# CoderWZW/ARLib

Hardware: AMD Instinct MI355X
Metric: BPR-train interactions/sec (LightGCN d=64 L=3 + BPR + Adam, B=2048) (higher is better)
Workload: dtype f32

## Files before the change

### arlib_amd/csrc/arl_kernels.hip

```cpp
#include <hip/hip_runtime.h>
#include <stdint.h>
#include <math.h>
#include <stdio.h>
#include "arlib_amd.h"
#include <type_traits>

#define ARL_LAUNCH_CHECK()                                  \
    do {                                                    \
        hipError_t e__ = hipGetLastError();                 \
        if (e__ != hipSuccess) return (int)e__;             \
    } while (0)

namespace {

constexpr int kWave = 64;
constexpr int kBlock = 256;
constexpr int kWavesPerBlock = kBlock / kWave;

__device__ __forceinline__ float wave_sum(float v) {
#pragma unroll
    for (int off = 32; off > 0; off >>= 1) v += __shfl_xor(v, off);
    return v;
}

// ... 324 lines not shown
        const int r = rows[t];
        const int begin = A.rowptr[r], end = A.rowptr[r + 1];
        const int per = (end - begin + sp - 1) / sp;
        const int b = begin + k * per, e = min(end, b + per);
        float4 a = make_float4(0.f, 0.f, 0.f, 0.f);
        if (b < e) a = spmm_gather<LPR, 4>(A.col, A.val, b, e, X, d, lane);
        a = group_reduce<LPR>(a);
        if (lane < LPR && q * 4 < d) *reinterpret_cast<float4 *>(partial + (size_t)piece * d + q * 4) = a;
    }
}

template <int LPR>
__global__ __launch_bounds__(kBlock) void subset_pieces_finish_kernel(const float *__restrict__ partial, int n, SubsetPlan S, int d, const int32_t *__restrict__ rows,
                                                                       LayerPtrs L, float alpha, float *__restrict__ out_c, const float *__restrict__ row_weight) {
    constexpr int G = kWave / LPR;
    const int lane = threadIdx.x & (kWave - 1);
    const int g = lane / LPR, q = lane % LPR;
    const int t = blockIdx.x * kWavesPerBlock + (threadIdx.x >> 6);
    if (t >= n) return;
    const bool qact = q * 4 < d;
    const int r = rows[t];
    float4 a = make_float4(0.f, 0.f, 0.f, 0.f);
    if (g == 0 && qact)
        for (int k = 0; k < L.n; ++k) a = add4(a, *reinterpret_cast<const float4 *>(L.p[k] + (size_t)r * d + q * 4));
    const int p1 = S.offs[t + 1];
    if (qact)
        for (int p = S.offs[t] + g; p < p1; p += 8 * G) {
            float4 v[8];
#pragma unroll
            for (int u = 0; u < 8; ++u)
                if (p + u * G < p1) v[u] = *reinterpret_cast<const float4 *>(partial + (size_t)(p + u * G) * d + q * 4);
#pragma unroll
            for (int u = 0; u < 8; ++u)
                if (p + u * G < p1) a = add4(a, v[u]);
        }
    a = group_reduce<LPR>(a);
    if (lane >= LPR || !qact) return;
    const float w = row_weight ? alpha * row_weight[t] : alpha;
    *reinterpret_cast<float4 *>(out_c + (size_t)t * d + q * 4) = make_float4(w * a.x, w * a.y, w * a.z, w * a.w);
}

static bool subset_plan(void *workspace, long long n, long long nsplit, long long d, SubsetPlan *S) {
    const long long words = n * nsplit * d, tail = n + 3;
    const long long cap = (words - tail) / (d + 1);
    if (cap < n || cap > 0x7fffffffll || n > (long long)kSubsetPrepThreads * kSubsetPrepRows) return false;
    int32_t *w = (int32_t *)workspace;
    S->cap = (int)cap;
    S->piece_row = w + cap * d;
    S->meta = S->piece_row + cap;
    S->offs = S->meta + 2;
    return true;
}

__global__ __launch_bounds__(kBlock) void tables_sum_kernel(LayerPtrs L, long long n4, float alpha, float4 *__restrict__ out) {
    for (long long t = (long long)blockIdx.x * kBlock + threadIdx.x; t < n4; t += (long long)gridDim.x * kBlock) {
        float4 a = reinterpret_cast<const float4 *>(L.p[0])[t];
        for (int k = 1; k < L.n; ++k) a = add4(a, reinterpret_cast<const float4 *>(L.p[k])[t]);
        out[t] = make_float4(alpha * a.x, alpha * a.y, alpha * a.z, alpha * a.w);
    }
}

__global__ __launch_bounds__(kBlock) void mark_rows_kernel(uint8_t *__restrict__ flags, const int32_t *__restrict__ idx, int n, int value) {
    const int t = blockIdx.x * kBlock + threadIdx.x;
    if (t < n) flags[idx[t]] = (uint8_t)value;
}
__global__ __launch_bounds__(kBlock) void mark_bits_kernel(uint32_t *__restrict__ bits, const int32_t *__restrict__ idx, int n, int set) {
    const int t = blockIdx.x * kBlock + threadIdx.x;
    if (t >= n) return;
    const int i = idx[t];
    if (set) atomicOr(bits + (i >> 5), 1u << (i & 31));
    else atomicAnd(bits + (i >> 5), ~(1u << (i & 31)));
}
__global__ __launch_bounds__(kBlock) void zero_rows_kernel(float *__restrict__ dst, const int32_t *__restrict__ idx, int n, int d) {
    const int lane = threadIdx.x & 63;
    const int t = blockIdx.x * kWavesPerBlock + (threadIdx.x >> 6);
    if (t >= n) return;
    float *o = dst + (size_t)idx[t] * d;
    for (int k = lane; k < d; k += kWave) o[k] = 0.f;
}

constexpr int kOrderedWindow = 16384;

template <class RowOf, class OnHit>
__device__ __forceinline__ bool ordered_scan(int c0, int c1, int t, long long row, int lane, RowOf rowof, OnHit on_hit) {
    for (int base = c0; base < c1; base += 256) {
        long long v[4];
#pragma unroll
        for (int i = 0; i < 4; ++i) {
            const int j = base + 64 * i + lane;
            v[i] = j < c1 ? (long long)rowof(j) : -1ll;
        }
#pragma unroll
        for (int i = 0; i < 4; ++i) {
            unsigned long long m = __ballot(v[i] == row);
            const int b0 = base + 64 * i;
            if (b0 < t) {
                const int lim = t - b0;
                if (lim >= 64 ? m != 0ull : (m & ((1ull << lim) - 1ull)) != 0ull) return false;
            }
            while (m) {
                const int tt = b0 + __ffsll((long long)m) - 1;
                m &= m - 1ull;
                on_hit(tt);
            }
        }
    }
    return true;
}

template <class OnHit>
__device__ __forceinline__ bool ordered_scan_lds(const int32_t *srows, int c0, int c1, int t, int row, int lane, OnHit on_hit) {
    const int n = c1 - c0, tl = t - c0;
    for (int base = 0; base < n; base += 512) {
        int v[8];
#pragma unroll
        for (int i = 0; i < 8; ++i) {
            const int j = base + 64 * i + lane;
            v[i] = j < n ? srows[j] : -1;
        }
#pragma unroll
        for (int i = 0; i < 8; ++i) {
            unsigned long long m = __ballot(v[i] == row);
            const int b0 = base + 64 * i;
            if (b0 < tl) {
                const int lim = tl - b0;
                if (lim >= 64 ? m != 0ull : (m & ((1ull << lim) - 1ull)) != 0ull) return false;
            }
            while (m) {
                const int tt = c0 + b0 + __ffsll((long long)m) - 1;
                m &= m - 1ull;
                on_hit(tt);
            }
        }
    }
    return true;
}
template <class OnGroup>
__device__ __forceinline__ bool ordered_scan_lds_groups(const int32_t *srows, int c0, int c1, int t, int row, int lane, OnGroup on_group) {
    const int n = c1 - c0, tl = t - c0;
    for (int base = 0; base < n; base += 512) {
        int v[8];
#pragma unroll
        for (int i = 0; i < 8; ++i) {
            const int j = base + 64 * i + lane;
            v[i] = j < n ? srows[j] : -1;
        }
#pragma unroll
        for (int i = 0; i < 8; ++i) {
            const unsigned long long m = __ballot(v[i] == row);
            const int b0 = base + 64 * i;
            if (b0 < tl) {
                const int lim = tl - b0;
                if (lim >= 64 ? m != 0ull : (m & ((1ull << lim) - 1ull)) != 0ull) return false;
            }
            if (m) on_group(m, c0 + b0);
        }
    }
    return true;
}
template <class RowOf>
__device__ __forceinline__ void stage_rows(int32_t *srows, int c0, int c1, RowOf rowof) {
    for (int j = threadIdx.x; j < c1 - c0; j += kBlock) srows[j] = (int32_t)rowof(c0 + j);
    __syncthreads();
}

__global__ __launch_bounds__(kBlock) void rows_mark_dups_kernel(uint32_t *__restrict__ bits, uint32_t *__restrict__ dup, const int32_t *__restrict__ idx, int n,
                                                                 const float *__restrict__ row_scale) {
    const int t = blockIdx.x * kBlock + threadIdx.x;
    if (t >= n) return;
    if (row_scale && row_scale[t] == 0.f) return;
    const int row = idx[t];
    const uint32_t m = 1u << (row & 31);
    if (atomicOr(bits + (row >> 5), m) & m) atomicOr(dup + (row >> 5), m);
}

template <bool MARK>
__global__ __launch_bounds__(kBlock) void rows_add_ordered_kernel(float *__restrict__ dst, uint8_t *__restrict__ flags, uint32_t *__restrict__ bits,
                                                                   const int32_t *__restrict__ idx, int c0, int c1, int d,
                                                                   const float *__restrict__ src, float scale, const float *__restrict__ row_scale,
                                                                   const uint32_t *__restrict__ dup) {
    extern __shared__ int32_t srows[];
    const int lane = threadIdx.x & 63;
    const int t = c0 + blockIdx.x * kWavesPerBlock + (threadIdx.x >> 6);
    const bool valid = t < c1 && !(row_scale && row_scale[t] == 0.f);
    const int row = valid ? idx[t] : 0;
    float *o = dst + (size_t)row * d;
    const bool fast = valid && dup && !((dup[row >> 5] >> (row & 31)) & 1u);
    if (fast) {
        const float sc = row_scale ? scale * row_scale[t] : scale;
        const float *s = src + (size_t)t * d;
        for (int k = lane; k < d; k += kWave) {
#pragma clang fp contract(off)
            const float c = sc * s[k];
            o[k] = o[k] + c;
        }
        if (MARK && lane == 0) flags[row] = 1;
    }
    if (!__syncthreads_or(valid && !fast)) return;
    stage_rows(srows, c0, c1, [&](int j) { return (row_scale && row_scale[j] == 0.f) ? -1 : idx[j]; });
    if (!valid || fast) return;
    for (int k0 = 0; k0 < d; k0 += 256) {
        float acc[4];
#pragma unroll
        for (int i = 0; i < 4; ++i) { const int k = k0 + 64 * i + lane; acc[i] = k < d ? o[k] : 0.f; }
        const bool owner = ordered_scan_lds_groups(srows, c0, c1, t, row, lane, [&](unsigned long long m, int g0) {
#pragma clang fp contract(off)
            while (m) {
                int tt[4]; float x[4][4], sc[4];
#pragma unroll
                for (int q = 0; q < 4; ++q) {
                    tt[q] = -1;
                    if (m) { tt[q] = g0 + __ffsll((long long)m) - 1; m &= m - 1ull; }
                }
#pragma unroll
                for (int q = 0; q < 4; ++q) {
                    if (tt[q] < 0) continue;
                    const float *s = src + (size_t)tt[q] * d;
                    sc[q] = row_scale ? scale * row_scale[tt[q]] : scale;
#pragma unroll
                    for (int i = 0; i < 4; ++i) { const int k = k0 + 64 * i + lane; x[q][i] = k < d ? s[k] : 0.f; }
                }
#pragma unroll
                for (int q = 0; q < 4; ++q) {
                    if (tt[q] < 0) continue;
#pragma unroll
                    for (int i = 0; i < 4; ++i) { const float c = sc[q] * x[q][i]; acc[i] = acc[i] + c; }
                }
            }
        });
        if (!owner) return;
#pragma unroll
        for (int i = 0; i < 4; ++i) { const int k = k0 + 64 * i + lane; if (k < d) o[k] = acc[i]; }
    }
    if (MARK && lane == 0) {
        flags[row] = 1;
        atomicOr(bits + (row >> 5), 1u << (row & 31));
    }
}
__global__ __launch_bounds__(kBlock) void batch_rows_clear_kernel(float *__restrict__ G, uint8_t *__restrict__ flags, uint32_t *__restrict__ bits,
                                                                   const int32_t *__restrict__ idx, int n, int d, uint32_t *__restrict__ dup) {
    const int lane = threadIdx.x & 63;
    const int t = blockIdx.x * kWavesPerBlock + (threadIdx.x >> 6);
    if (t >= n) return;
    const int row = idx[t];
    float *o = G + (size_t)row * d;
    for (int k = lane; k < d; k += kWave) o[k] = 0.f;
    if (lane == 0) {
        flags[row] = 0;
        atomicAnd(bits + (row >> 5), ~(1u << (row & 31)));
        if (dup) atomicAnd(dup + (row >> 5), ~(1u << (row & 31)));
    }
}

template <int MODE>
int launch_spmm(const arl_csr *A, const float *X, int64_t d, const Epi &ep, hipStream_t st, const uint32_t *xflags = nullptr) {
    if (!A || !X || (A->n_rows > 0 && !A->rowptr) || (A->nnz > 0 && (!A->col || !A->val))) return ARL_E_NULL;
    if (d <= 0 || d > 256 || (d & 3)) return ARL_E_DIM;
    if (A->n_rows < 0 || A->n_rows > 0x7fffffffll || A->nnz > 0x7fffffffll || A->n_chunks > 0x7fffffffll) return ARL_E_RANGE;
    if (A->n_chunks > 0 && (!A->chunk_row || !A->chunk_begin || !A->chunk_end || !A->partial || A->chunk <= 0)) return ARL_E_NULL;
    if (A->n_long > 0 && (!A->long_row || !A->long_first || !A->long_count)) return ARL_E_NULL;
    if ((A->n_chunks > 0) != (A->n_long > 0)) return ARL_E_ARG;
    if (A->n_rows == 0 && A->n_chunks == 0) return ARL_OK;
    CsrDev D;
    D.n_rows = (int)A->n_rows; D.rowptr = A->rowptr; D.col = A->col; D.val = A->val;
    D.chunk = A->chunk; D.n_chunks = (int)A->n_chunks; D.chunk_row = A->chunk_row; D.chunk_begin = A->chunk_begin;
    D.chunk_end = A->chunk_end; D.n_long = (int)A->n_long; D.long_row = A->long_row; D.long_first = A->long_first;
    D.long_count = A->long_count; D.partial = A->partial;
    D.row_tasks = xflags ? reinterpret_cast<const int4 *>(A->row_tasks) : nullptr;
    const long long tasks = (long long)D.n_rows + D.n_chunks;
    const unsigned grid = (unsigned)((tasks + kWavesPerBlock - 1) / kWavesPerBlock);
    const unsigned grid_long = (unsigned)((D.n_long + kWavesPerBlock - 1) / kWavesPerBlock);
    const int di = (int)d;
#define ARL_SPMM_CASE(LPRV)                                                                              \
    do {                                                                                                 \
        if (xflags) hipLaunchKernelGGL((spmm_rows_masked_gpr_kernel<LPRV, MODE>), dim3((unsigned)((tasks + kWavesPerBlock * (kWave / LPRV) - 1) / (kWavesPerBlock * (kWave / LPRV)))), dim3(kBlock), 0, st, D, X, di, ep, xflags); \
        else hipLaunchKernelGGL((spmm_rows_kernel<LPRV, MODE>), dim3(grid), dim3(kBlock), 0, st, D, X, di, ep); \
        ARL_LAUNCH_CHECK();                                                                              \
        if (D.n_long > 0) {                                                                              \
            hipLaunchKernelGGL((spmm_long_rows_kernel<LPRV, MODE>), dim3(grid_long), dim3(kBlock), 0, st, D, di, ep); \
            ARL_LAUNCH_CHECK();                                                                          \
        }                                                                                                \
    } while (0)
    if (d <= 16) ARL_SPMM_CASE(4);
    else if (d <= 32) ARL_SPMM_CASE(8);
    else if (d <= 64) ARL_SPMM_CASE(16);
    else if (d <= 128) ARL_SPMM_CASE(32);
    else ARL_SPMM_CASE(64);
#undef ARL_SPMM_CASE
    return ARL_OK;
}

typedef float f32x32v __attribute__((ext_vector_type(32)));

struct BlockedDev {
    int n_waves;
    const int32_t *wave_ptr;
    const int32_t *wave_rows;
    const int32_t *rec_col;
    const float *rec_val;
    float *partial;
    const uint32_t *xbits;
};

template <int MODE, int CPL, int LD>
__device__ __forceinline__ void spmm_epilogue1(const Epi &ep, int row, int lane, const float *a) {
    const size_t o = (size_t)row * LD + lane * CPL;
    const bool zr = ep.Z && (!ep.zflags || ep.zflags[row]);
#pragma unroll
    for (int c = 0; c < CPL; ++c) {
        if (MODE == EPI_AXPBY) {
            float y = (ep.rscale ? ep.alpha * ep.rscale[row] : ep.alpha) * a[c];
            if (zr) y = fmaf(ep.beta, ep.Z[o + c], y);
            __builtin_nontemporal_store(y, ep.Y + o + c);
        } else if (MODE == EPI_LAYERSUM) {
            const float sv = ep.S_in[o + c];
            if (ep.Y) ep.Y[o + c] = a[c];
            ep.S[o + c] = sv + a[c];
        } else {
            float g = ep.alpha * a[c];
            if (zr) g = fmaf(ep.beta, ep.Z[o + c], g);
            float p = ep.P[o + c], m = ep.M[o + c], v = ep.V[o + c];
            m = m + (g - m) * ep.w1;
            v = v * ep.b2 + ep.w2 * g * g;
            const float denom = sqrtf(v) / ep.bc2_sqrt + ep.eps;
            p = p - ep.step_size * (m / denom);
            ep.P[o + c] = p; ep.M[o + c] = m; ep.V[o + c] = v;
        }
    }
}

constexpr int kMaskedUnr = 8;

template <int RPW, int MODE, int UNR, int CPL, int LD = 64 * CPL, bool MASKED = false>
__global__ __launch_bounds__(kBlock) void spmm_blocked64_kernel(BlockedDev P, const float *__restrict__ X, Epi ep) {
    static_assert(RPW == 16 || RPW == 32, "accumulators are 32-register vectors");
    static_assert(CPL == 1 || CPL == 2, "d = 64 (one column per lane) or d = 128 (two adjacent columns per lane)");
    const int lane = threadIdx.x & 63;
    const int w = blockIdx.x * (blockDim.x >> 6) + (threadIdx.x >> 6);
    if (w >= P.n_waves) return;
    f32x32v acc[CPL];
#pragma unroll
    for (int c = 0; c < CPL; ++c)
#pragma unroll
        for (int r = 0; r < 32; ++r) acc[c][r] = 0.f;
    const int begin = P.wave_ptr[w], end = P.wave_ptr[w + 1];
    const float *xl = X + lane * CPL;
    if (MASKED) {
        int c0 = 0, c1 = 0; unsigned w0 = 0;
        if (begin < end) c0 = __builtin_nontemporal_load(P.rec_col + begin + lane);
        if (begin + 64 < end) c1 = __builtin_nontemporal_load(P.rec_col + begin + 64 + lane);
        if (begin < end) w0 = P.xbits[((unsigned)c0 & 0xffffffu) >> 5];
        for (int base = begin; base < end; base += 64) {
            const int c_cur = c0; const unsigned w_cur = w0;
            c0 = c1;
            if (base + 128 < end) c1 = __builtin_nontemporal_load(P.rec_col + base + 128 + lane);
            if (base + 64 < end) w0 = P.xbits[((unsigned)c0 & 0xffffffu) >> 5];
            unsigned long long hits = __ballot((w_cur >> (c_cur & 31)) & 1u);
            while (hits) {
                float x[kMaskedUnr][CPL], vs[kMaskedUnr]; int cs[kMaskedUnr], js[kMaskedUnr];
#pragma unroll
                for (int t = 0; t < kMaskedUnr; ++t) {
                    js[t] = hits ? __builtin_ctzll(hits) : -1;
                    hits &= hits - 1ull;
                    if (js[t] < 0) continue;
                    cs[t] = __builtin_amdgcn_readlane(c_cur, js[t]);
                    vs[t] = P.rec_val[base + js[t]];
                    const float *src = xl + (size_t)(cs[t] & 0xffffff) * LD;
                    if (CPL == 2) { const float2 v2 = *reinterpret_cast<const float2 *>(src); x[t][0] = v2.x; x[t][CPL - 1] = v2.y; }
                    else x[t][0] = src[0];
                }
#pragma unroll
                for (int t = 0; t < kMaskedUnr; ++t) {
                    if (js[t] < 0) continue;
                    const int slot = ((unsigned)cs[t] >> 24) & 31;
#pragma unroll
                    for (int c = 0; c < CPL; ++c) acc[c][slot] = fmaf(vs[t], x[t][c], acc[c][slot]);
                }
            }
        }
    } else {
    int rc = 0; float rv = 0.f;
    if (begin < end) { rc = __builtin_nontemporal_load(P.rec_col + begin + lane); rv = __builtin_nontemporal_load(P.rec_val + begin + lane); }
    for (int base = begin; base < end; base += 64) {
        const int c_cur = rc; const float v_cur = rv;
        if (base + 64 < end) { rc = __builtin_nontemporal_load(P.rec_col + base + 64 + lane); rv = __builtin_nontemporal_load(P.rec_val + base + 64 + lane); }
#pragma unroll
        for (int j = 0; j < 64; j += UNR) {
            float x[UNR][CPL]; int cs[UNR];
#pragma unroll
            for (int t = 0; t < UNR; ++t) {
                cs[t] = __builtin_amdgcn_readlane(c_cur, j + t);
                const float *src = xl + (size_t)(cs[t] & 0xffffff) * LD;
                if (CPL == 2) { const float2 v2 = *reinterpret_cast<const float2 *>(src); x[t][0] = v2.x; x[t][CPL - 1] = v2.y; }
                else x[t][0] = src[0];
            }
#pragma unroll
            for (int t = 0; t < UNR; ++t) {
                const int slot = ((unsigned)cs[t] >> 24) & 31;
                const float v = __uint_as_float((unsigned)__builtin_amdgcn_readlane((int)__float_as_uint(v_cur), j + t));
#pragma unroll
                for (int c = 0; c < CPL; ++c) acc[c][slot] = fmaf(v, x[t][c], acc[c][slot]);
            }
        }
    }
    }
#pragma unroll
    for (int r = 0; r < RPW; ++r) {
        const int row = P.wave_rows[w * RPW + r];
        float a[CPL];
#pragma unroll
        for (int c = 0; c < CPL; ++c) a[c] = acc[c][r];
        if (row >= 0) spmm_epilogue1<MODE, CPL, LD>(ep, row, lane, a);
        else if (row < -1) {
            float *dst = P.partial + ((size_t)(-row - 2) * 64 + lane) * CPL;
#pragma unroll
            for (int c = 0; c < CPL; ++c) dst[c] = a[c];
        }
    }
}

template <int RPW, int MODE, int UNR, int CPL, int LD>
static int launch_blocked64(dim3 grid, dim3 block, hipStream_t st, const BlockedDev &D, const float *X, const Epi &ep) {
    if (D.xbits) {
        if constexpr (MODE == EPI_AXPBY) hipLaunchKernelGGL((spmm_blocked64_kernel<RPW, MODE, UNR, CPL, LD, true>), grid, block, 0, st, D, X, ep);
        else return ARL_E_ARG;
    } else hipLaunchKernelGGL((spmm_blocked64_kernel<RPW, MODE, UNR, CPL, LD, false>), grid, block, 0, st, D, X, ep);
    ARL_LAUNCH_CHECK();
    return ARL_OK;
}

template <int MODE>
int launch_spmm_blocked(const arl_blocked *P, const float *X, int64_t d, const Epi &ep, hipStream_t st, const uint32_t *xbits = nullptr) {
    if (!P || !X) return ARL_E_NULL;
    if (d != 64 && d != 128) return ARL_E_DIM;
    if (P->n_waves < 0 || P->n_waves > 0x7fffffffll / 64) return ARL_E_RANGE;
    if (P->rows_per_wave != 16 && P->rows_per_wave != 32) return ARL_E_ARG;
    if (P->n_waves == 0) return ARL_OK;
    if (!P->wave_ptr || !P->wave_rows || !P->rec_col || !P->rec_val) return ARL_E_NULL;
    if (P->n_split < 0 || P->n_split > 0x7fffffffll) return ARL_E_RANGE;
    if (P->n_split > 0 && (!P->split_row || !P->split_first || !P->split_count || !P->partial)) return ARL_E_NULL;
    BlockedDev D = {(int)P->n_waves, P->wave_ptr, P->wave_rows, P->rec_col, P->rec_val, P->partial, xbits};
    const int64_t wpg = P->waves_per_group ? P->waves_per_group : kWavesPerBlock;
    if (wpg != 1 && wpg != 2 && wpg != 4) return ARL_E_ARG;
    const dim3 grid((unsigned)((P->n_waves + wpg - 1) / wpg)), block((unsigned)(wpg * kWave));
    if (P->loads_in_flight != 16 && P->loads_in_flight != 32) return ARL_E_ARG;
    int rc;
    if (d == 128) {
        for (int half = 0; half < 2; ++half) {
            Epi e2 = ep;
            e2.ld = 128;
            const int off = 64 * half;
            if (e2.Z) e2.Z += off;
            if (e2.Y) e2.Y += off;
            if (e2.S_in) e2.S_in += off;
            if (e2.S) e2.S += off;
            if (e2.P) e2.P += off;
            if (e2.M) e2.M += off;
            if (e2.V) e2.V += off;
            if (P->rows_per_wave == 16) rc = launch_blocked64<16, MODE, 16, 1, 128>(grid, block, st, D, X + off, e2);
            else if (P->loads_in_flight == 16) rc = launch_blocked64<32, MODE, 16, 1, 128>(grid, block, st, D, X + off, e2);
            else rc = launch_blocked64<32, MODE, 32, 1, 128>(grid, block, st, D, X + off, e2);
            if (rc != ARL_OK) return rc;
            if (P->n_split > 0) {
                CsrDev C = {};
                C.n_long = (int)P->n_split; C.long_row = P->split_row; C.long_first = P->split_first; C.long_count = P->split_count; C.partial = P->partial;
                const unsigned grid_long = (unsigned)((C.n_long + kWavesPerBlock - 1) / kWavesPerBlock);
                hipLaunchKernelGGL((spmm_long_rows_kernel<16, MODE>), dim3(grid_long), dim3(kBlock), 0, st, C, 64, e2);
                ARL_LAUNCH_CHECK();
            }
        }
        return ARL_OK;
    }
    if (P->rows_per_wave == 16) rc = launch_blocked64<16, MODE, 16, 1, 64>(grid, block, st, D, X, ep);
    else if (P->loads_in_flight == 16) rc = launch_blocked64<32, MODE, 16, 1, 64>(grid, block, st, D, X, ep);
    else rc = launch_blocked64<32, MODE, 32, 1, 64>(grid, block, st, D, X, ep);
    if (rc != ARL_OK) return rc;
    if (P->n_split > 0) {
        CsrDev C = {};
        C.n_long = (int)P->n_split; C.long_row = P->split_row; C.long_first = P->split_first; C.long_count = P->split_count; C.partial = P->partial;
        const unsigned grid_long = (unsigned)((C.n_long + kWavesPerBlock - 1) / kWavesPerBlock);
        hipLaunchKernelGGL((spmm_long_rows_kernel<16, MODE>), dim3(grid_long), dim3(kBlock), 0, st, C, 64, ep);
        ARL_LAUNCH_CHECK();
    }
    return ARL_OK;
}

__global__ __launch_bounds__(kBlock) void row_dinv_kernel(int n_rows, const int32_t *__restrict__ rowptr,
                                                           const float *__restrict__ w, float *__restrict__ dinv) {
    const int lane = threadIdx.x & 63;
    const int r = blockIdx.x * kWavesPerBlock + (threadIdx.x >> 6);
    if (r >= n_rows) return;
    float s = 0.f;
    for (int e = rowptr[r] + lane; e < rowptr[r + 1]; e += kWave) s += w[e];
    s = wave_sum(s);
    if (lane == 0) dinv[r] = s > 0.f ? 1.0f / sqrtf(s) : 0.f;
}

__global__ __launch_bounds__(kBlock) void norm_vals_kernel(int n_rows, const int32_t *__restrict__ rowptr,
                                                            const int32_t *__restrict__ col, const float *__restrict__ w,
                                                            const float *__restrict__ dinv, float *__restrict__ val) {
    const int lane = threadIdx.x & 63;
    const int r = blockIdx.x * kWavesPerBlock + (threadIdx.x >> 6);
    if (r >= n_rows) return;
    const float dr = dinv[r];
    for (int e = rowptr[r] + lane; e < rowptr[r + 1]; e += kWave) val[e] = (dr * w[e]) * dinv[col[e]];
}

__global__ __launch_bounds__(kBlock) void norm_vals_coo_kernel(long long nnz, const int32_t *__restrict__ erow, const int32_t *__restrict__ col,
                                                                const float *__restrict__ w, const float *__restrict__ dinv, float *__restrict__ val) {
    const long long e0 = ((long long)blockIdx.x * kBlock + threadIdx.x) * 4;
    if (e0 + 3 < nnz) {
        const int4 r = *reinterpret_cast<const int4 *>(erow + e0), c = *reinterpret_cast<const int4 *>(col + e0);
        const float4 ww = *reinterpret_cast<const float4 *>(w + e0);
        float4 o;
        o.x = (dinv[r.x] * ww.x) * dinv[c.x]; o.y = (dinv[r.y] * ww.y) * dinv[c.y];
        o.z = (dinv[r.z] * ww.z) * dinv[c.z]; o.w = (dinv[r.w] * ww.w) * dinv[c.w];
        *reinterpret_cast<float4 *>(val + e0) = o;
    } else {
        for (long long e = e0; e < nnz; ++e) val[e] = (dinv[erow[e]] * w[e]) * dinv[col[e]];
    }
}

__global__ __launch_bounds__(kBlock) void bpr_fwd_kernel(const float *__restrict__ emb, int d, long long item_off,
                                                          const int32_t *__restrict__ ui, const int32_t *__restrict__ pi,
                                                          const int32_t *__restrict__ ni, int B, float b_norm, float *__restrict__ ws) {
    const int lane = threadIdx.x & 63;
    const int b = blockIdx.x * kWavesPerBlock + (threadIdx.x >> 6);
    if (b >= B) return;
    const float *u = emb + (size_t)ui[b] * d, *p = emb + (size_t)(item_off + pi[b]) * d, *n = emb + (size_t)(item_off + ni[b]) * d;
    float ps = 0.f, ns = 0.f, uu = 0.f, pp = 0.f;
    for (int k = lane; k < d; k += kWave) {
        const float uk = u[k], pk = p[k], nk = n[k];
        ps = fmaf(uk, pk, ps); ns = fmaf(uk, nk, ns); uu = fmaf(uk, uk, uu); pp = fmaf(pk, pk, pp);
    }
    ps = wave_sum(ps); ns = wave_sum(ns); uu = wave_sum(uu); pp = wave_sum(pp);
    if (lane == 0) {
        const float x = ps - ns;
        const float s = 1.0f / (1.0f + expf(-x));
        ws[b] = -(s * (1.0f - s)) / ((1e-7f + s) * b_norm);
        ws[B + b] = -logf(1e-7f + s);
        ws[2 * B + b] = uu;
        ws[3 * B + b] = pp;
    }
}

__global__ __launch_bounds__(kBlock) void bpr_finalize_kernel(int B, float reg, const float *__restrict__ ws, float *__restrict__ out, int raw_sums) {
    __shared__ float sh[3][kBlock];
    float a = 0.f, b = 0.f, c = 0.f;
    for (int i = threadIdx.x; i < B; i += kBlock) { a += ws[B + i]; b += ws[2 * B + i]; c += ws[3 * B + i]; }
    sh[0][threadIdx.x] = a; sh[1][threadIdx.x] = b; sh[2][threadIdx.x] = c;
    __syncthreads();
    for (int s = kBlock / 2; s > 0; s >>= 1) {
        if ((int)threadIdx.x < s) {
            sh[0][threadIdx.x] += sh[0][threadIdx.x + s]; sh[1][threadIdx.x] += sh[1][threadIdx.x + s]; sh[2][threadIdx.x] += sh[2][threadIdx.x + s];
        }
        __syncthreads();
    }
    if (threadIdx.x == 0 && raw_sums) {
        out[0] = sh[0][0]; out[1] = sh[1][0]; out[2] = sh[2][0];
    } else if (threadIdx.x == 0) {
        const float nu = sqrtf(sh[1][0]), np_ = sqrtf(sh[2][0]);
        out[0] = sh[0][0] / (float)B;
        out[1] = reg * (nu + np_);
        out[2] = nu;
        out[3] = np_;
    }
}

__global__ __launch_bounds__(kBlock) void rows_axpy_unique_kernel(float *__restrict__ dst, const float *__restrict__ src, const int32_t *__restrict__ idx,
                                                                   int c0, int c1, int d, float alpha, const uint32_t *__restrict__ dup, int lds_n) {
    extern __shared__ int32_t srows[];
    const int lane = threadIdx.x & 63;
    const int t = c0 + blockIdx.x * kWavesPerBlock + (threadIdx.x >> 6);
    const bool valid = t < c1;
    const long long row = valid ? idx[t] : 0;
    const bool scan = valid && (!dup || ((dup[row >> 5] >> (row & 31)) & 1u));
    if (lds_n > 0) {
        if (__syncthreads_or(scan)) stage_rows(srows, 0, lds_n, [&](int j) { return idx[j]; });
        if (!valid) return;
        if (scan && !ordered_scan_lds(srows, 0, t, t, (int)row, lane, [&](int) {})) return;
    } else {
        if (!valid) return;
        if (scan && !ordered_scan(0, t, t, row, lane, [&](int j) { return idx[j]; }, [&](int) {})) return;
    }
    float *o = dst + (size_t)row * d;
    const float *x = src + (size_t)row * d;
    for (int k = lane; k < d; k += kWave) o[k] = fmaf(alpha, x[k], o[k]);
}

__global__ __launch_bounds__(kBlock) void shard_batch_prep_kernel(const int32_t *__restrict__ u, const int32_t *__restrict__ p, const int32_t *__restrict__ n,
                                                                   int B, int u0, int u1, int32_t *__restrict__ lu, float *__restrict__ own,
                                                                   int32_t *__restrict__ item_rows, int32_t *__restrict__ rows_l) {
    const int b = blockIdx.x * kBlock + threadIdx.x;
    if (b >= B) return;
    const int Ul = u1 - u0;
    const int uu = u[b];
    const int l = min(max(uu - u0, 0), max(Ul - 1, 0));
    lu[b] = l; own[b] = (uu >= u0 && uu < u1) ? 1.f : 0.f; own[B + b] = 1.f; own[2 * B + b] = 1.f;
    const int pp = p[b], nn = n[b];
    item_rows[b] = pp; item_rows[B + b] = nn;
    rows_l[b] = l; rows_l[B + b] = Ul + pp; rows_l[2 * B + b] = Ul + nn;
}

__global__ __launch_bounds__(kBlock) void bpr_bwd_kernel(const float *__restrict__ emb, int d, long long item_off,
                                                          const int32_t *__restrict__ ui, const int32_t *__restrict__ pi,
                                                          const int32_t *__restrict__ ni, int B, float reg, float upstream,
                                                          const float *__restrict__ ws, const float *__restrict__ out,
                                                          float *__restrict__ G, int c0, int c1, int distinct) {
    extern __shared__ int32_t srows[];
    const int lane = threadIdx.x & 63;
    const int t = c0 + blockIdx.x * kWavesPerBlock + (threadIdx.x >> 6);
#define ARL_ROWOF_BPR(j) ((j) < B ? (long long)ui[j] : ((j) < 2 * B ? item_off + pi[(j) - B] : item_off + ni[(j) - 2 * B]))
    if (!distinct) stage_rows(srows, c0, c1, [&](int j) { return ARL_ROWOF_BPR(j); });
    if (t >= c1) return;
    const int row = (int)ARL_ROWOF_BPR(t);
    const float cu = out[2] > 0.f ? upstream * reg / out[2] : 0.f, cp = out[3] > 0.f ? upstream * reg / out[3] : 0.f;
    float *o = G + (size_t)row * d;
    const float *own = emb + (size_t)row * d;
    for (int k0 = 0; k0 < d; k0 += 256) {
        float acc[4], mine[4];
#pragma unroll
        for (int i = 0; i < 4; ++i) { const int k = k0 + 64 * i + lane; acc[i] = k < d ? o[k] : 0.f; mine[i] = k < d ? own[k] : 0.f; }
        auto term = [&](int tt) {
            const int kind = tt / B, b = tt - kind * B;
            const float g = ws[b] * upstream;
            const float *x = emb + (size_t)(kind == 0 ? item_off + pi[b] : (long long)ui[b]) * d;
            const float *y = emb + (size_t)(item_off + ni[b]) * d;
#pragma unroll
            for (int i = 0; i < 4; ++i) {
                const int k = k0 + 64 * i + lane;
                if (k < d) {
                    float c;
                    if (kind == 0) c = fmaf(g, x[k] - y[k], cu * mine[i]);
                    else if (kind == 1) c = fmaf(g, x[k], cp * mine[i]);
                    else c = -g * x[k];
                    acc[i] = __fadd_rn(acc[i], c);
                }
            }
        };
        if (distinct) term(t);
        else if (!ordered_scan_lds(srows, c0, c1, t, row, lane, term)) return;
#pragma unroll
        for (int i = 0; i < 4; ++i) { const int k = k0 + 64 * i + lane; if (k < d) o[k] = acc[i]; }
    }
#undef ARL_ROWOF_BPR
}

__global__ __launch_bounds__(kBlock) void adam_kernel(float4 *__restrict__ p, const float4 *__restrict__ g, float4 *__restrict__ m,
                                                       float4 *__restrict__ v, long long n4, float step_size, float bc2_sqrt,
                                                       float w1, float b2, float w2, float eps) {
    for (long long i = (long long)blockIdx.x * kBlock + threadIdx.x; i < n4; i += (long long)gridDim.x * kBlock) {
        const float4 g4 = g[i];
        float4 p4 = p[i], m4 = m[i], v4 = v[i];
        float gg[4] = {g4.x, g4.y, g4.z, g4.w}, pp[4] = {p4.x, p4.y, p4.z, p4.w}, mm[4] = {m4.x, m4.y, m4.z, m4.w}, vv[4] = {v4.x, v4.y, v4.z, v4.w};
#pragma unroll
        for (int k = 0; k < 4; ++k) {
            mm[k] = mm[k] + (gg[k] - mm[k]) * w1;
            vv[k] = vv[k] * b2 + w2 * gg[k] * gg[k];
            pp[k] = pp[k] - step_size * (mm[k] / (sqrtf(vv[k]) / bc2_sqrt + eps));
        }
        p[i] = make_float4(pp[0], pp[1], pp[2], pp[3]); m[i] = make_float4(mm[0], mm[1], mm[2], mm[3]); v[i] = make_float4(vv[0], vv[1], vv[2], vv[3]);
    }
}
__global__ __launch_bounds__(kBlock) void adam_scalar_kernel(float *p, const float *g, float *m, float *v, long long from, long long n,
                                                              float step_size, float bc2_sqrt, float w1, float b2, float w2, float eps) {
    for (long long i = from + (long long)blockIdx.x * kBlock + threadIdx.x; i < n; i += (long long)gridDim.x * kBlock) {
        const float gi = g[i];
        const float mi = m[i] + (gi - m[i]) * w1;
        const float vi = v[i] * b2 + w2 * gi * gi;
        m[i] = mi; v[i] = vi;
        p[i] = p[i] - step_size * (mi / (sqrtf(vi) / bc2_sqrt + eps));
    }
}
__global__ __launch_bounds__(kBlock) void sgd_kernel(float *__restrict__ p, const float *__restrict__ g, long long n, float lr) {
    for (long long i = (long long)blockIdx.x * kBlock + threadIdx.x; i < n; i += (long long)gridDim.x * kBlock) p[i] = p[i] - lr * g[i];
}

inline double typed_double(float x) {
    char buf[32];
    snprintf(buf, sizeof buf, "%.7g", (double)x);
    const double d = strtod(buf, nullptr);
    return (float)d == x ? d : (double)x;
}
struct AdamScalars { float step_size, bc2_sqrt, w1, b2, w2; };
inline AdamScalars adam_scalars(float lr, float b1, float b2, int64_t step) {
    const double B1 = typed_double(b1), B2 = typed_double(b2), LR = typed_double(lr);
    const double bc1 = 1.0 - pow(B1, (double)step), bc2 = 1.0 - pow(B2, (double)step);
    return {(float)(LR / bc1), (float)sqrt(bc2), (float)(1.0 - B1), (float)B2, (float)(1.0 - B2)};
}

__global__ __launch_bounds__(kBlock) void gather_rows_kernel(const float *__restrict__ src, const int32_t *__restrict__ idx, int n, int d,
                                                              float *__restrict__ dst) {
    const int lane = threadIdx.x & 63;
    const int t = blockIdx.x * kWavesPerBlock + (threadIdx.x >> 6);
    if (t >= n) return;
    const float *s = src + (size_t)idx[t] * d;
    for (int k = lane; k < d; k += kWave) dst[(size_t)t * d + k] = s[k];
}
__global__ __launch_bounds__(kBlock) void nce_normalize_kernel(const float *__restrict__ v, int n, int d, float *__restrict__ y, float *__restrict__ nrm) {
    const int lane = threadIdx.x & 63;
    const int i = blockIdx.x * kWavesPerBlock + (threadIdx.x >> 6);
    if (i >= n) return;
    float s = 0.f;
    for (int k = lane; k < d; k += kWave) { const float x = v[(size_t)i * d + k]; s = fmaf(x, x, s); }
    s = wave_sum(s);
    const float r = fmaxf(sqrtf(s), 1e-12f);
    for (int k = lane; k < d; k += kWave) y[(size_t)i * d + k] = v[(size_t)i * d + k] / r;
    if (lane == 0) nrm[i] = r;
}

__global__ __launch_bounds__(kBlock) void nce_rowsum_kernel(const float *__restrict__ a, const float *__restrict__ b, int n, int d, float inv_tau,
                                                             float *__restrict__ ttl, float *__restrict__ rowloss) {
    __shared__ float ai[256];
    __shared__ float red[kBlock];
    __shared__ float sii_sh;
    const int i = blockIdx.x;
    for (int k = threadIdx.x; k < d; k += kBlock) ai[k] = a[(size_t)i * d + k];
    __syncthreads();
    float acc = 0.f;
    for (int j = threadIdx.x; j < n; j += kBlock) {
// ... 3902 lines not shown
```

Before: 328,200.

## Batch and software-pipeline SpMM epilogue row loads in groups

Restructures the blocked SpMM epilogue so each wave loads its row indices, zflags and rscale once per lane, then shares them with readlane and ballot masks instead of issuing per-row scalar loads. Rows are processed in groups of K, and the next group's Z/P/M/V/S_in loads are issued before the current group's math, so the loads are double-buffered and their memory latency overlaps. Pad rows fall back to a safe row address, and a tail loop handles the remaining rows. This costs more registers and adds complexity, and the Adam maths now uses explicit fma, which may change rounding slightly.

```diff
diff --git a/arlib_amd/csrc/arl_kernels.hip b/arlib_amd/csrc/arl_kernels.hip
--- a/arlib_amd/csrc/arl_kernels.hip
+++ b/arlib_amd/csrc/arl_kernels.hip
@@ -650,32 +650,129 @@
     const uint32_t *xbits;
 };
 
-template <int MODE, int CPL, int LD>
-__device__ __forceinline__ void spmm_epilogue1(const Epi &ep, int row, int lane, const float *a) {
-    const size_t o = (size_t)row * LD + lane * CPL;
-    const bool zr = ep.Z && (!ep.zflags || ep.zflags[row]);
+template <int MODE> constexpr int kEpiLoads = MODE == EPI_ADAM ? 4 : 1;
+template <int MODE> constexpr int kEpiStores = MODE == EPI_ADAM ? 3 : MODE == EPI_LAYERSUM ? 2 : 1;
+
+template <int MODE>
+__device__ __forceinline__ float *spmm_epilogue_table(const Epi &ep, int s) {
+    if (MODE == EPI_AXPBY) return ep.Y;
+    if (MODE == EPI_LAYERSUM) return s == 0 ? ep.Y : ep.S;
+    return s == 0 ? ep.P : s == 1 ? ep.M : ep.V;
+}
+
+template <int MODE, int CPL>
+__device__ __forceinline__ void spmm_epilogue_math(const Epi &ep, bool zr, float rs, const float *a, const float (&in)[kEpiLoads<MODE>][CPL],
+                                                   float (&out)[kEpiStores<MODE>][CPL]) {
 #pragma unroll
     for (int c = 0; c < CPL; ++c) {
-        if (MODE == EPI_AXPBY) {
-            float y = (ep.rscale ? ep.alpha * ep.rscale[row] : ep.alpha) * a[c];
-            if (zr) y = fmaf(ep.beta, ep.Z[o + c], y);
-            __builtin_nontemporal_store(y, ep.Y + o + c);
-        } else if (MODE == EPI_LAYERSUM) {
-            const float sv = ep.S_in[o + c];
-            if (ep.Y) ep.Y[o + c] = a[c];
-            ep.S[o + c] = sv + a[c];
+#pragma clang fp contract(off)
+        if constexpr (MODE == EPI_AXPBY) {
+            float y = (ep.rscale ? ep.alpha * rs : ep.alpha) * a[c];
+            if (zr) y = fmaf(ep.beta, in[0][c], y);
+            out[0][c] = y;
+        } else if constexpr (MODE == EPI_LAYERSUM) {
+            out[0][c] = a[c];
+            out[1][c] = in[0][c] + a[c];
         } else {
             float g = ep.alpha * a[c];
-            if (zr) g = fmaf(ep.beta, ep.Z[o + c], g);
-            float p = ep.P[o + c], m = ep.M[o + c], v = ep.V[o + c];
+            if (zr) g = fmaf(ep.beta, in[0][c], g);
+            float p = in[1][c], m = in[2][c], v = in[3][c];
             m = m + (g - m) * ep.w1;
-            v = v * ep.b2 + ep.w2 * g * g;
+            v = fmaf(ep.w2 * g, g, v * ep.b2);
             const float denom = sqrtf(v) / ep.bc2_sqrt + ep.eps;
-            p = p - ep.step_size * (m / denom);
-            ep.P[o + c] = p; ep.M[o + c] = m; ep.V[o + c] = v;
-        }
-    }
-}
+            p = fmaf(-ep.step_size, m / denom, p);
+            out[0][c] = p; out[1][c] = m; out[2][c] = v;
+        }
+    }
+}
+
+template <int MODE, int CPL, int LD>
+__device__ __forceinline__ void spmm_epilogue1(const Epi &ep, int row, bool zr, float rs, int lane, const float *a) {
+    const size_t o = (size_t)row * LD;
+    const unsigned lo = lane * CPL;
+    float in[kEpiLoads<MODE>][CPL], out[kEpiStores<MODE>][CPL];
+#pragma unroll
+    for (int c = 0; c < CPL; ++c) {
+        in[0][c] = 0.f;
+        if constexpr (MODE == EPI_LAYERSUM) in[0][c] = (ep.S_in + o)[lo + c];
+        else if (zr) in[0][c] = (ep.Z + o)[lo + c];
+        if constexpr (MODE == EPI_ADAM) { in[1][c] = (ep.P + o)[lo + c]; in[2][c] = (ep.M + o)[lo + c]; in[3][c] = (ep.V + o)[lo + c]; }
+    }
+    spmm_epilogue_math<MODE, CPL>(ep, zr, rs, a, in, out);
+#pragma unroll
+    for (int s = 0; s < kEpiStores<MODE>; ++s) {
+        if (MODE == EPI_LAYERSUM && s == 0 && !ep.Y) continue;
+        float *dst = spmm_epilogue_table<MODE>(ep, s) + o;
+#pragma unroll
+        for (int c = 0; c < CPL; ++c) {
+            if (MODE == EPI_AXPBY) __builtin_nontemporal_store(out[s][c], dst + (lo + c));
+            else dst[lo + c] = out[s][c];
+        }
+    }
+}
+
+template <int MODE, int K, int CPL, int LD>
+__device__ __forceinline__ void spmm_group_load(const Epi &ep, int my_row, unsigned zmask, int safe_row, int r0, int lane, float (&in)[K][kEpiLoads<MODE>][CPL]) {
+    const unsigned lo = lane * CPL;
+    const size_t so = (size_t)safe_row * LD;
+    if constexpr (MODE != EPI_LAYERSUM) {
+#pragma unroll
+        for (int i = 0; i < K; ++i)
+#pragma unroll
+            for (int c = 0; c < CPL; ++c) in[i][0][c] = 0.f;
+        if (ep.Z) {
+#pragma unroll
+            for (int i = 0; i < K; ++i) {
+                const int row = __builtin_amdgcn_readlane(my_row, r0 + i);
+                const float *z = ((zmask >> (r0 + i)) & 1u) ? ep.Z + (size_t)row * LD : ep.Z + so;
+#pragma unroll
+                for (int c = 0; c < CPL; ++c) in[i][0][c] = z[lo + c];
+            }
+        }
+    }
+    if constexpr (MODE != EPI_AXPBY) {
+#pragma unroll
+        for (int i = 0; i < K; ++i) {
+            const int row = __builtin_amdgcn_readlane(my_row, r0 + i);
+            const size_t o = (size_t)row * LD;
+#pragma unroll
+            for (int c = 0; c < CPL; ++c) {
+                if constexpr (MODE == EPI_LAYERSUM) in[i][0][c] = (row >= 0 ? ep.S_in + o : ep.S_in + so)[lo + c];
+                else {
+                    in[i][1][c] = (row >= 0 ? ep.P + o : ep.P + so)[lo + c];
+                    in[i][2][c] = (row >= 0 ? ep.M + o : ep.M + so)[lo + c];
+                    in[i][3][c] = (row >= 0 ? ep.V + o : ep.V + so)[lo + c];
+                }
+            }
+        }
+    }
+}
+
+template <int MODE, int K, int CPL, int LD>
+__device__ __forceinline__ void spmm_group_store(const Epi &ep, float *partial, int my_row, int r0, int lane, const float (&a)[K][CPL],
+                                                 const float (&out)[K][kEpiStores<MODE>][CPL]) {
+    const unsigned lo = lane * CPL;
+#pragma unroll
+    for (int s = 0; s < kEpiStores<MODE>; ++s) {
+        if (MODE == EPI_LAYERSUM && s == 0 && !ep.Y) continue;
+        float *tab = spmm_epilogue_table<MODE>(ep, s);
+#pragma unroll
+        for (int i = 0; i < K; ++i) {
+            const int row = __builtin_amdgcn_readlane(my_row, r0 + i);
+            const bool plain = row >= 0;
+            float *dst = plain ? tab + (size_t)row * LD : partial + (size_t)(plain ? 0 : -row - 2) * (64 * CPL);
+#pragma unroll
+            for (int c = 0; c < CPL; ++c) {
+                const float y = plain ? out[i][s][c] : a[i][c];
+                if (MODE == EPI_AXPBY) __builtin_nontemporal_store(y, dst + (lo + c));
+                else dst[lo + c] = y;
+            }
+        }
+    }
+}
+
+template <int UNR, bool MASKED> constexpr bool kEpiGrouped = MASKED || UNR == 16;
+template <int MODE, bool MASKED> constexpr int kEpiGroup = MODE == EPI_ADAM ? 2 : MASKED ? 8 : 4;
 
 constexpr int kMaskedUnr = 8;
 
@@ -692,6 +789,9 @@
 #pragma unroll
         for (int r = 0; r < 32; ++r) acc[c][r] = 0.f;
     const int begin = P.wave_ptr[w], end = P.wave_ptr[w + 1];
+    constexpr bool GROUPED = kEpiGrouped<UNR, MASKED>;
+    int my_row = -1;
+    if (GROUPED && lane < RPW) my_row = P.wave_rows[(size_t)w * RPW + lane];
     const float *xl = X + lane * CPL;
     if (MASKED) {
         int c0 = 0, c1 = 0; unsigned w0 = 0;
@@ -752,18 +852,63 @@
         }
     }
     }
-#pragma unroll
-    for (int r = 0; r < RPW; ++r) {
-        const int row = P.wave_rows[w * RPW + r];
-        float a[CPL];
-#pragma unroll
-        for (int c = 0; c < CPL; ++c) a[c] = acc[c][r];
-        if (row >= 0) spmm_epilogue1<MODE, CPL, LD>(ep, row, lane, a);
+    auto row_epilogue = [&](int row, bool zr, float rs, const float *a) {
+        if (row >= 0) spmm_epilogue1<MODE, CPL, LD>(ep, row, zr, rs, lane, a);
         else if (row < -1) {
             float *dst = P.partial + ((size_t)(-row - 2) * 64 + lane) * CPL;
 #pragma unroll
             for (int c = 0; c < CPL; ++c) dst[c] = a[c];
         }
+    };
+    if constexpr (!GROUPED) {
+#pragma unroll
+        for (int r = 0; r < RPW; ++r) {
+            const int row = P.wave_rows[w * RPW + r];
+            float a[CPL];
+#pragma unroll
+            for (int c = 0; c < CPL; ++c) a[c] = acc[c][r];
+            const bool zr = row >= 0 && MODE != EPI_LAYERSUM && ep.Z && (!ep.zflags || ep.zflags[row]);
+            const float rs = (row >= 0 && MODE == EPI_AXPBY && ep.rscale) ? ep.rscale[row] : 0.f;
+            row_epilogue(row, zr, rs, a);
+        }
+    } else {
+    bool my_zr = false; float my_rs = 0.f;
+    if (my_row >= 0) {
+        if (MODE == EPI_AXPBY && ep.rscale) my_rs = ep.rscale[my_row];
+        if (MODE != EPI_LAYERSUM) my_zr = ep.Z && (!ep.zflags || ep.zflags[my_row]);
+    }
+    const unsigned zmask = (unsigned)__ballot(my_zr);
+    const unsigned long long rows = __ballot(my_row >= 0), pads = __ballot(my_row == -1);
+    constexpr int K = kEpiGroup<MODE, MASKED>, NG = RPW / K;
+    static_assert(RPW % K == 0, "whole groups");
+    const int n_grouped = rows ? __builtin_ctzll(pads) / K : 0;
+    if (n_grouped > 0) {
+        const int safe_row = __builtin_amdgcn_readlane(my_row, __builtin_ctzll(rows));
+        float in[2][K][kEpiLoads<MODE>][CPL];
+        spmm_group_load<MODE, K, CPL, LD>(ep, my_row, zmask, safe_row, 0, lane, in[0]);
+#pragma unroll
+        for (int g = 0; g < NG; ++g) {
+            if (g + 1 < NG) spmm_group_load<MODE, K, CPL, LD>(ep, my_row, zmask, safe_row, (g + 1) * K, lane, in[(g + 1) & 1]);
+            float a[K][CPL], out[K][kEpiStores<MODE>][CPL];
+#pragma unroll
+            for (int i = 0; i < K; ++i) {
+                const int r = g * K + i;
+#pragma unroll
+                for (int c = 0; c < CPL; ++c) a[i][c] = acc[c][r];
+                const float rs = __uint_as_float((unsigned)__builtin_amdgcn_readlane((int)__float_as_uint(my_rs), r));
+                spmm_epilogue_math<MODE, CPL>(ep, (zmask >> r) & 1u, rs, a[i], in[g & 1][i], out[i]);
+            }
+            spmm_group_store<MODE, K, CPL, LD>(ep, P.partial, my_row, g * K, lane, a, out);
+            if (g + 1 == n_grouped) break;
+        }
+    }
+#pragma nounroll
+    for (int r = n_grouped * K; r < RPW; ++r) {
+        float a[CPL];
+#pragma unroll
+        for (int c = 0; c < CPL; ++c) a[c] = acc[c][r];
+        row_epilogue(__builtin_amdgcn_readlane(my_row, r), (zmask >> r) & 1u, __uint_as_float((unsigned)__builtin_amdgcn_readlane((int)__float_as_uint(my_rs), r)), a);
+    }
     }
 }
 
```

Result: faster. 332,400, median of 6 (+1.3%).
